# cambyse/po-rrt

Measured on AMD Instinct MI355X. Metric: RRT node-expansions/sec on map_benchmark.pgm, higher is better.
Workload: dtype f64

## Files before the change

### po_rrt_amd/csrc/porrt_device.hpp

```cpp
#pragma once
#include <hip/hip_runtime.h>
#include <stdint.h>
#include <string>
#include <vector>
#include "../../include/porrt_hip.h"

namespace porrt {

template <int NEV>
struct ScopedEvents {
    hipEvent_t e[NEV];
    ScopedEvents() { for (int i = 0; i < NEV; ++i) e[i] = nullptr; }
    hipError_t create() {
        for (int i = 0; i < NEV; ++i) { const hipError_t r = hipEventCreate(&e[i]); if (r != hipSuccess) return r; }
        return hipSuccess;
    }
    ~ScopedEvents() { for (int i = 0; i < NEV; ++i) if (e[i]) (void)hipEventDestroy(e[i]); }
    ScopedEvents(const ScopedEvents &) = delete;
    ScopedEvents &operator=(const ScopedEvents &) = delete;
};

template <class Launch, class GoingOn>
static int sweep_to_fixpoint(hipStream_t stream, uint32_t *flags, size_t rows, int cur, Launch &&launch, GoingOn &&going_on, const char *who,
                             uint64_t &sweeps, std::string &err) {
// ... 66 lines not shown
    uint32_t pend_cnt, pool_n;
    uint32_t n_deferred, pend_lo;
    uint32_t n_losers;
    uint32_t kd_snap;
    uint32_t dbg[4];
    uint32_t clone_n;
    uint32_t clone_k[64];
    uint32_t coop_bar;
    uint32_t coop_filed;
    uint32_t coop_abort;
    uint32_t sched_stop;
    uint32_t sched_iter;
    uint32_t n_lca;
    uint32_t lca_next;
    unsigned long long tim[16];
};

#ifdef PORRT_TIMING
#define PORRT_T0() unsigned long long t__0 = wall_clock64()
#define PORRT_TACC(rc, slot)                                                                          \
    do {                                                                                              \
        const unsigned long long t__1 = wall_clock64();                                               \
        if ((threadIdx.x & 63u) == 0u) { atomicAdd(&(rc).cnt->tim[slot], t__1 - t__0); atomicAdd(&(rc).cnt->tim[(slot) + 8], 1ull); } \
        t__0 = t__1;                                                                                  \
    } while (0)
#else
#define PORRT_T0() do {} while (0)
#define PORRT_TACC(rc, slot) do {} while (0)
#endif
#ifndef PORRT_TIMING_FROM
// ... 757 lines not shown
#else
template <class T> using HitRow = T __attribute__((address_space(1))) *;
template <class T> using LdsPtr = T *;
#endif

__device__ __forceinline__ uint32_t region_of(const RunConst &rc, double x, double y) {
    int cx, cy;
    rep_cell(rc, x, y, kRG, cx, cy);
    return (uint32_t)(cy * kRG + cx);
}

__device__ __forceinline__ double disc_radius(double bound_d2, double qx, double qy) {
    return sqrt(bound_d2) * (1.0 + 1e-9) + 1e-12 * (1.0 + fabs(qx) + fabs(qy));
}

template <bool BUF = false, class Visit>
__device__ __forceinline__ void scan_disc(const RunConst &rc, uint32_t b, double qx, double qy, double rho, uint32_t N, uint32_t lane, Visit visit,
                                          uint32_t skip_region = 0xFFFFFFFFu, uint32_t share = 0u, uint32_t nshare = 1u) {
    int cx0, cy0, cx1, cy1;
    rep_cell(rc, qx - rho, qy - rho, kRG, cx0, cy0);
    rep_cell(rc, qx + rho, qy + rho, kRG, cx1, cy1);
    const uint32_t x0 = uni((uint32_t)cx0), y0 = uni((uint32_t)cy0);
    const uint32_t w = uni((uint32_t)(cx1 - cx0 + 1)), nreg = w * uni((uint32_t)(cy1 - cy0 + 1));
    if (nreg * 16u > N) {
        [[maybe_unused]] auto gx = as_global(rc.nx), gy = as_global(rc.ny);
        for (uint32_t j0 = share * 128u; j0 < N; j0 += nshare * 128u) {
            double x[2], y[2];
#pragma unroll
            for (int u = 0; u < 2; ++u) {
                const uint32_t j = j0 + 64u * u + lane;
                if constexpr (BUF) {
                    x[u] = g_at(rc.nx, (j < N ? j : 0u) * 8u);
                    y[u] = g_at(rc.ny, (j < N ? j : 0u) * 8u);
                } else {
                    x[u] = gx[j < N ? j : 0u];
                    y[u] = gy[j < N ? j : 0u];
                }
            }
#pragma unroll
            for (int u = 0; u < 2; ++u)
                if (j0 + 64u * u < N) visit(x[u], y[u], (int)(j0 + 64u * u + lane), j0 + 64u * u + lane < N);
        }
        return;
    }
    auto gcnt = as_global(rc.rg_cnt) + (b & 1u) * kRegions;
    auto gdir = as_global(rc.rg_dir);
    [[maybe_unused]] auto gxy = as_global(reinterpret_cast<const dbl2 *>(rc.pg_xy));
    [[maybe_unused]] auto gid = as_global(rc.pg_id);
    [[maybe_unused]] PageBuf pb;
    if constexpr (BUF) pb = page_buf(rc);
    for (uint32_t r0 = 0; r0 < nreg; r0 += 64) {
        const uint32_t r = r0 + lane;
        uint32_t reg = 0, cnt = 0;
        if (r < nreg) {
            const uint32_t ry = r / w;
            reg = (y0 + ry) * kRG + x0 + (r - ry * w);
            cnt = reg == skip_region ? 0u : gcnt[reg];
        }
        const uint32_t npg = (uint32_t)__popcll(__ballot(cnt > 0u));
        if (__ballot(cnt >= npg || cnt > kPage) == 0ull && npg > 1u) {
            if (nshare > 1u && r % nshare != share) cnt = 0u;
            uint32_t cmax = cnt;
            for (int off = 32; off > 0; off >>= 1) {
                const uint32_t o = __shfl_xor(cmax, off);
                cmax = o > cmax ? o : cmax;
            }
            cmax = uni(cmax);
            for (uint32_t s0 = 0; s0 < cmax; s0 += 2) {
                dbl2 v[2];
                int id[2];
#pragma unroll
                for (int u = 0; u < 2; ++u) {
                    if constexpr (BUF) {
                        const uint32_t at = s0 + u < cnt ? reg * kPage + s0 + u : kNoSlot;
                        v[u] = page_xy(pb, at);
                        id[u] = page_id(pb, at);
                    } else {
                        const uint32_t sl = s0 + u < cnt ? s0 + u : 0u;
                        v[u] = gxy[(size_t)reg * kPage + sl];
                        id[u] = gid[(size_t)reg * kPage + sl];
                    }
                }
                if constexpr (BUF) __atomic_signal_fence(__ATOMIC_SEQ_CST);
#pragma unroll
                for (int u = 0; u < 2; ++u)
                    if (s0 + u < cmax) visit(v[u].x, v[u].y, id[u], s0 + u < cnt);
            }
            continue;
        }
        uint32_t page = reg;
        for (uint32_t j = 0;; ++j) {
            unsigned long long m = __ballot(cnt > j * kPage);
            if (!m) break;
            if (nshare > 1u) m = __ballot(cnt > j * kPage && (r + j) % nshare == share);
            if (j && cnt > j * kPage) page = gdir[(size_t)reg * rc.rg_maxp + j];
            while (m) {
                uint32_t pg[2], pc[2];
#pragma unroll
                for (int u = 0; u < 2; ++u) {
                    pg[u] = 0; pc[u] = 0;
                    if (m) {
                        const uint32_t l = (uint32_t)__builtin_ctzll(m);
                        m &= m - 1;
                        pg[u] = (uint32_t)__builtin_amdgcn_readlane((int)page, (int)l);
                        const uint32_t c = (uint32_t)__builtin_amdgcn_readlane((int)cnt, (int)l) - j * kPage;
                        pc[u] = c < kPage ? c : kPage;
                    }
                }
                dbl2 v[2];
                int id[2];
#pragma unroll
                for (int u = 0; u < 2; ++u) {
                    const bool ld = lane < pc[u];
                    if constexpr (BUF) {
                        const uint32_t at = ld ? pg[u] * kPage + lane : kNoSlot;
                        v[u] = page_xy(pb, at);
                        id[u] = page_id(pb, at);
                    } else {
                        v[u] = ld ? gxy[(size_t)pg[u] * kPage + lane] : dbl2{0.0, 0.0};
                        id[u] = ld ? gid[(size_t)pg[u] * kPage + lane] : -1;
                    }
                }
                if constexpr (BUF) __atomic_signal_fence(__ATOMIC_SEQ_CST);
#pragma unroll
                for (int u = 0; u < 2; ++u)
                    if (pc[u]) visit(v[u].x, v[u].y, id[u], lane < pc[u]);
            }
        }
    }
}

template <bool PTO>
__device__ __forceinline__ void near_sample(const RunConst &rc, uint32_t b, uint32_t i0, uint32_t vwords, uint32_t k, uint32_t lane) {
    const uint32_t N = uni(as_global(rc.n_at)[b]);
    const double sqx = uni_d(as_global(rc.sx)[i0 + k]), sqy = uni_d(as_global(rc.sy)[i0 + k]);
    uint32_t world = 0;
    if (PTO) world = uni(as_global(rc.sworld)[i0 + k]);
    const double INF = __longlong_as_double(0x7FF0000000000000ll);
    double bestD = INF;
    int best = 0x7FFFFFFF;
    const double T2 = rc.rad_T2[N + (rc.mode == 1 ? 1u : 0u)];
// ... 547 lines not shown
        }
        return v;
    }
};

struct GlobalList {
    static constexpr bool kCompact = false;
    GPTR(const int) cid;
    GPTR(const dbl2) cxy;
    GPTR(double) cval;
    GPTR(const double) gdA;
    __device__ __forceinline__ int id(uint32_t a) const { return cid[a]; }
    __device__ __forceinline__ void xy(uint32_t a, double &x, double &y) const { const dbl2 v = cxy[a]; x = v.x; y = v.y; }
    __device__ __forceinline__ double val(uint32_t a) const { return cval[a]; }
    __device__ __forceinline__ void set_val(uint32_t a, double v) const { cval[a] = v; }
    __device__ __forceinline__ void set_dA(uint32_t, double) const {}
    __device__ __forceinline__ double dA(uint32_t, int j) const { return gdA[j]; }
};
__device__ __forceinline__ GlobalList global_list(const RunConst &rc, uint32_t b, uint32_t k) {
    GlobalList L;
    L.cid = as_global((const int *)rc.cand_id) + cand_off(rc, b, k);
    L.cxy = as_global(reinterpret_cast<const dbl2 *>(rc.cand_xy)) + cand_off(rc, b, k);
    L.cval = as_global(rc.cand_val) + cand_val_off(rc, b, k);
    L.gdA = as_global((const double *)rc.distA);
    return L;
}
#ifndef PORRT_LDS_HITS
#define PORRT_LDS_HITS 80
#endif
constexpr uint32_t kLdsHits = PORRT_LDS_HITS;
// ... 18 lines not shown
    static constexpr bool kCompact = true;
    HitRow<int> sid;
    HitRow<dbl2> sxy;
    HitRow<double> sd;
    HitRow<int> out_id;
    HitRow<double> out_val;
    GPTR(uint32_t) out_cnt;
    uint32_t out_cap;
    __device__ __forceinline__ int id(uint32_t a) const { return sid[a]; }
    __device__ __forceinline__ void xy(uint32_t a, double &x, double &y) const { const dbl2 v = sxy[a]; x = v.x; y = v.y; }
    __device__ __forceinline__ double val(uint32_t a) const { return sxy[a].x; }
    __device__ __forceinline__ void set_val(uint32_t a, double v) const { sxy[a].x = v; }
    __device__ __forceinline__ void set_dA(uint32_t, double) const {}
    __device__ __forceinline__ double dA(uint32_t a, int) const { return sd[a]; }
};

struct NoNearestSearch { __device__ int operator()() const { return 0; } };
template <class TeamT, class ListT, class Grid, class NNF = NoNearestSearch>
__device__ void connect_rrt_sample(const RunConst &rc, const TeamT &tm, const ListT &L, const Grid &grid, uint32_t b, uint32_t k, uint32_t id,
                                   double px, double py, uint32_t cnt, uint32_t &err, const uint32_t *clone_ids = nullptr, uint32_t n_clone = 0,
                                   int clr_known = -1, NNF nearest_search = NNF(), uint32_t swap = 0) {
    const uint32_t tl = tm.tl(), TS = TeamT::kSize;
    const int goal_kind = rc.goal_kind;
    auto gdA = as_global(swap ? rc.distB : rc.distA);
    const double INF = __longlong_as_double(0x7FF0000000000000ll);

    PORRT_T0();
    double bt = INF;
    int bj = 0x7FFFFFFF;
    uint32_t nvalid = 0, leq = 0;
// ... 261 lines not shown
            }
            if (tl == 0) *L.out_cnt = n_out;
        }
        PORRT_TACC_S(rc, 7);
        return;
    } else {
    if (j0 >= 0) {
        double out = -1.0;
        if (nvalid != 0 && cost0 >= 0.0 && j0 != best) {
            const double via = dnew + cost0;
            if (via < dA0) {
                g_atomic_min(gdB + j0, f64_bits(via));
                out = via;
            }
        }
        L.set_val(tl, out);
    }
    for (uint32_t a = tl + TS; a < cnt; a += TS) {
        const double cost = L.val(a);
        const int j = L.id(a);
        double out = -1.0;
        if (nvalid != 0 && cost >= 0.0 && j != best) {
            const double via = dnew + cost;
            if (via < L.dA(a, j)) {
                g_atomic_min(gdB + j, f64_bits(via));
                out = via;
            }
        }
        L.set_val(a, out);
    }
    }
}

constexpr uint32_t kHeavyCand = 256;

template <bool LDSGRID>
__device__ __forceinline__ void connect_block(const RunConst &rc, uint32_t b, uint32_t nb, uint32_t vwords, uint32_t bx, uint8_t *lds_tiles, double *s_d, int *s_i,
                                              uint32_t *s_heavy, uint32_t swap = 0) {
    const uint32_t lane = threadIdx.x & 63u, wv = threadIdx.x >> 6;
    const uint32_t k = uni(bx * kConnectWaves + wv);
    const uint32_t qo = q_off(rc, b);
    const bool active = k < nb && as_global(rc.q_vid)[qo + (k < nb ? k : 0)] >= 0;
    const uint32_t cnt = active ? cand_count(rc, b, k) : 0u;
    const bool heavy = active && cnt > kHeavyCand;
// ... 1549 lines not shown
```

### po_rrt_amd/csrc/porrt_engine.hip

```cpp
#include "../../include/porrt_hip.h"
#include "porrt_host.hpp"
#include "porrt_device.hpp"
#include "porrt_group.hpp"
#include "porrt_belief.hpp"
#include "porrt_dp.hpp"
#include "porrt_prm.hpp"
#include "porrt_edges.hpp"
#include "porrt_refine.hpp"
#include "porrt_refine_batch.hpp"
#include "porrt_reparent.hpp"
#include "porrt_qmdp.hpp"
#include "porrt_policy_graph.hpp"
#include "porrt_join.hpp"
#include "porrt_mm_recipe.hpp"

#include <algorithm>
#include <functional>
#include <chrono>
#include <cmath>
#include <cstdio>
#include <cstring>
#include <string>
#include <system_error>
#include <mutex>
// ... 81 lines not shown
    bool opt_graph = true;
    uint32_t opt_kd_group = 0;
    bool opt_kd_after = false;
    int opt_kd_inline = 0;
    int opt_kd_lazy = 1;
    uint32_t opt_claim_threads = 0;
    int opt_host_ranks = 1;
    int opt_compact = 1;
    uint32_t n_compactions = 0;
    int opt_kd_ride = 0;
    int opt_group_req = -1;
    uint32_t opt_early_wave = 0;
    uint32_t opt_conn_wg_waves = 1;
    bool opt_conn_riders_first = true;
    uint32_t opt_riders_fast = 1;
    uint32_t opt_nn_wg_waves = 4;
    uint32_t opt_commit_flat = 1;
    uint32_t opt_batch_streams = 0;
    int opt_pipeline = 4;
    std::vector<void *> dl_pin;
    std::vector<hipStream_t> dl_streams;
    std::vector<size_t> dl_pin_cap;
    hipStream_t dl_out_stream = nullptr;
    TreeOut *d_tree_out = nullptr;
    size_t d_tree_out_cap = 0;
    uint32_t opt_tree_out_blocks = 4;
    uint32_t opt_fetch_workers = 8;
    bool sub_eager = false;
    int last_launch_mode = 0;
    uint32_t sub_streams_tried = 0;
// ... 555 lines not shown
        return;
    }
    (void)hipEventRecord(ev_steered, stream);
    ev();
    if (GLn) {
        const uint32_t lazy = kd_lazy ? 1u : 0u;
        if (cx.opt_conn_wg_waves == 4u) {
            const uint32_t spb = 256u / GLc;
            const dim3 g2((nb + spb - 1) / spb + 2 + lazy, Q);
            const size_t dyn = conn2_wg4_lds_bytes(GLc);
            with_lanes(GLc, [&](auto gl) { hipLaunchKernelGGL(k_conn2_wg4<decltype(gl)::value>, g2, dim3(256), dyn, stream, rcp, b, nb, vwords, lazy, cx.opt_riders_fast); });
        } else {
            const uint32_t spb = 64u / GLc;
            const dim3 g2((nb + spb - 1) / spb, Q), gr(2 + lazy, Q);
            const size_t dyn = conn2_lds_bytes(GLc);
            if (cx.opt_conn_riders_first) hipLaunchKernelGGL(k_conn2_riders, gr, dim3(256), conn2_riders_lds_bytes(), stream, rcp, b, nb, vwords, lazy, cx.opt_riders_fast);
            with_lanes(GLc, [&](auto gl) { hipLaunchKernelGGL(k_conn2<decltype(gl)::value>, g2, dim3(64), dyn, stream, rcp, b, nb, vwords); });
            if (!cx.opt_conn_riders_first) hipLaunchKernelGGL(k_conn2_riders, gr, dim3(256), conn2_riders_lds_bytes(), stream, rcp, b, nb, vwords, lazy, cx.opt_riders_fast);
        }
    } else if (lds_bytes) hipLaunchKernelGGL(k_connect_rrt<true>, cgrid, cblock, lds_bytes, stream, rcp, b, nb, vwords);
    else hipLaunchKernelGGL(k_connect_rrt<false>, cgrid, cblock, 0, stream, rcp, b, nb, vwords);
    ev();
    commit_pend_b = b; commit_pend_nb = nb;
    kd_last_b = b; kd_last_nb = nb;
    side_active = true;
    if (!cx.opt_kd_after && !kd_lazy && b + 1 - kd_b0 >= kd_group) launch_kd_group();
}

static uint32_t launch_kd_claim(hipStream_t st, const RunConst *rcp, uint32_t Q, uint32_t b0, uint32_t ns, uint32_t K, uint32_t vwords, uint32_t threads) {
    const uint64_t nodes = (uint64_t)ns * K;
    if (Q == 1 && threads == 0) {
        if (nodes <= 2048u) { hipLaunchKernelGGL(k_kd_claim<2048>, dim3(1, 1), dim3(1024), 0, st, rcp, b0, ns, vwords); return kKdfClaimOne2048; }
        hipLaunchKernelGGL(k_kd_claim<kClaimMax>, dim3(1, 1), dim3(1024), 0, st, rcp, b0, ns, vwords);
// ... 4101 lines not shown

int porrt_get_option(const porrt_ctx *c, const char *name, int64_t *value) {
    if (!c || !name || !value) return PORRT_ERR_INVALID;
    if (!strcmp(name, "launch_mode")) *value = c->last_launch_mode;
    else if (!strcmp(name, "pipeline")) *value = c->seq.lag_on ? 4 : (c->seq.pipe_on ? 1 : 0);
    else if (!strcmp(name, "group_lanes")) *value = c->seq.opt_group;
    else if (!strcmp(name, "kd_lazy")) *value = c->seq.kd_lazy ? 1 : 0;
    else if (!strcmp(name, "kd_lca_steps")) *value = (int64_t)c->counters.lca_next;
    else if (!strcmp(name, "compactions")) *value = c->n_compactions;
    else if (!strcmp(name, "kd_built_after")) *value = c->seq.kd_built_after;
    else if (!strcmp(name, "kd_forms_run")) *value = c->seq.kd_forms_run;
    else if (!strcmp(name, "n_heavy")) *value = (int64_t)c->counters.n_heavy;
    else if (!strcmp(name, "conn_wg_waves")) *value = c->opt_conn_wg_waves;
    else if (!strcmp(name, "conn_riders_first")) *value = c->opt_conn_riders_first ? 1 : 0;
    else if (!strcmp(name, "riders_fast")) *value = c->opt_riders_fast;
    else if (!strncmp(name, "tim", 3) && name[3] >= '0' && name[3] <= '9' && atoi(name + 3) < 16) *value = (int64_t)c->counters.tim[atoi(name + 3)];
    else if (!strcmp(name, "nn_wg_waves")) *value = c->opt_nn_wg_waves;
    else if (!strcmp(name, "commit_flat")) *value = c->opt_commit_flat;
    else if (!strcmp(name, "cand_cap")) *value = c->opt_cand_cap;
    else if (!strcmp(name, "edge_per_node")) *value = (int64_t)c->edge_per_node;
    else if (!strcmp(name, "tie_pool_ids")) *value = (int64_t)c->tie_pool_ids;
    else if (!strcmp(name, "tie_pooled_ids")) *value = (int64_t)c->counters.pool_n;
    else if (!strcmp(name, "tie_records")) *value = (int64_t)c->counters.pend_cnt;
    else if (!strcmp(name, "dp_wide_rows")) *value = (int64_t)c->opt_dp_wide_rows;
    else if (!strcmp(name, "dp_levels")) *value = c->dp.valid ? (int64_t)c->dp.levels : 0;
    else if (!strcmp(name, "tamp_streams")) *value = c->opt_tamp_streams;
    else if (!strcmp(name, "tamp_wave")) *value = c->opt_tamp_wave;
    else if (!strcmp(name, "tamp_pool")) *value = c->opt_tamp_pool;
    else if (!strcmp(name, "tamp_search")) *value = c->opt_tamp_search;
    else if (!strcmp(name, "tamp_arena_states")) *value = (int64_t)c->opt_tamp_arena_states;
// ... 41 lines not shown
    }
    else if (!strcmp(name, "batch_streams")) c->opt_batch_streams = (uint32_t)std::max<int64_t>(0, std::min<int64_t>(value, 8));
    else if (!strcmp(name, "kd_after")) c->opt_kd_after = value != 0;
    else if (!strcmp(name, "kd_ride")) c->opt_kd_ride = value != 0;
    else if (!strcmp(name, "kd_lazy")) c->opt_kd_lazy = value == 2 ? 2 : (value != 0);
    else if (!strcmp(name, "kd_claim_threads")) { if (value != 0 && value != 256 && value != 512 && value != 1024) return PORRT_ERR_INVALID; c->opt_claim_threads = (uint32_t)value; }
    else if (!strcmp(name, "kd_inline")) c->opt_kd_inline = value != 0;
    else if (!strcmp(name, "compact_rows")) c->opt_compact = value != 0;
    else if (!strcmp(name, "fetch_workers")) c->opt_fetch_workers = (uint32_t)std::max<int64_t>(1, std::min<int64_t>(value, 32));
    else if (!strcmp(name, "tree_out_blocks")) c->opt_tree_out_blocks = (uint32_t)std::max<int64_t>(1, std::min<int64_t>(value, 1024));
    else if (!strcmp(name, "host_ranks")) { c->opt_host_ranks = value != 0; c->eo.tag = ~0ull; }
    else if (!strcmp(name, "early_wave_steps")) c->opt_early_wave = (uint32_t)std::max<int64_t>(0, std::min<int64_t>(value, 64));
    else if (!strcmp(name, "conn_wg_waves")) { if (value != 1 && value != 4) { c->set_err("conn_wg_waves: 1 or 4"); return PORRT_ERR_INVALID; } c->opt_conn_wg_waves = (uint32_t)value; }
    else if (!strcmp(name, "conn_riders_first")) c->opt_conn_riders_first = value != 0;
    else if (!strcmp(name, "riders_fast")) { if (value != 0 && value != 1) { c->set_err("riders_fast: 0 or 1"); return PORRT_ERR_INVALID; } c->opt_riders_fast = (uint32_t)value; }
    else if (!strcmp(name, "nn_wg_waves")) { if (value != 1 && value != 4) { c->set_err("nn_wg_waves: 1 or 4"); return PORRT_ERR_INVALID; } c->opt_nn_wg_waves = (uint32_t)value; }
    else if (!strcmp(name, "commit_flat")) { if (value != 0 && value != 1) { c->set_err("commit_flat: 0 or 1"); return PORRT_ERR_INVALID; } c->opt_commit_flat = (uint32_t)value; }
    else if (!strcmp(name, "kd_group")) c->opt_kd_group = (uint32_t)std::max<int64_t>(0, std::min<int64_t>(value, 8));
    else if (!strcmp(name, "tamp_streams")) { if (value != 0 && value != 1) { c->set_err("tamp_streams: 0 or 1"); return PORRT_ERR_INVALID; } c->opt_tamp_streams = (int)value; }
    else if (!strcmp(name, "tamp_wave")) { if (value < 1 || value > 65536) { c->set_err("tamp_wave: 1 .. 65536"); return PORRT_ERR_INVALID; } c->opt_tamp_wave = (uint32_t)value; }
    else if (!strcmp(name, "tamp_pool")) { if (value < 1 || value > 4096) { c->set_err("tamp_pool: 1 .. 4096"); return PORRT_ERR_INVALID; } c->opt_tamp_pool = (uint32_t)value; }
    else if (!strcmp(name, "tamp_arena_states")) { if (value < 1024 || value > (1ll << 31)) { c->set_err("tamp_arena_states: 1024 (one row's gather) .. 2^31"); return PORRT_ERR_INVALID; } c->opt_tamp_arena_states = (uint64_t)value; }
    else if (!strcmp(name, "tamp_search")) { if (value < 0 || value > 2) { c->set_err("tamp_search: 0 (BranchAndBound), 1 (AStar), 2 (BranchAndBoundMultipleViewPoints)"); return PORRT_ERR_INVALID; } c->opt_tamp_search = (int)value; }
    else if (!strcmp(name, "prm_rows")) { if (value < 1 || value > 4096) { c->set_err("prm_rows: 1 .. 4096"); return PORRT_ERR_INVALID; } c->opt_prm_rows = (uint32_t)value; }
    else if (!strcmp(name, "prm_xcd_rows")) c->opt_prm_xcd_rows = value != 0;
    else if (!strcmp(name, "policy_max_nodes")) { if (value < 1 || value > (int64_t)kPolMaxNodesLimit) { c->set_err("policy_max_nodes: 1 .. 2^24"); return PORRT_ERR_INVALID; } c->opt_policy_max_nodes = (uint32_t)value; }
    else if (!strcmp(name, "plan_batch_max_belief_nodes")) { if (value < 1 || value > (int64_t)kJoinBeliefNodesLimit) { c->set_err("plan_batch_max_belief_nodes: 1 .. 2^32 - 2"); return PORRT_ERR_INVALID; } c->opt_plan_batch_max_belief_nodes = (uint64_t)value; }
    else if (!strcmp(name, "plan_batch_host_ranks")) c->opt_plan_batch_host_ranks = value != 0;
    else if (!strcmp(name, "mm_plan_batch_max_nodes")) { if (value < 1 || value > (int64_t)kMmBatchNodesLimit) { c->set_err("mm_plan_batch_max_nodes: 1 .. 2^31 - 2"); return PORRT_ERR_INVALID; } c->opt_mm_plan_batch_max_nodes = (uint64_t)value; }
    else if (!strcmp(name, "policy_graph_max_pivots")) { if (value < 0 || value > (int64_t)0x7FFFFFFF) { c->set_err("policy_graph_max_pivots: 0 .. 2^31 - 1"); return PORRT_ERR_INVALID; } c->opt_policy_graph_max_pivots = (uint32_t)value; }
// ... 14 lines not shown
```

### po_rrt_amd/csrc/porrt_group.hpp

```cpp
#pragma once
#include "porrt_device.hpp"
#include "porrt_span.hpp"

namespace porrt {


struct GscanNothingBeside { __device__ __forceinline__ void operator()() const {} };
template <int GL, int R, bool WITHD, class Visit, class Beside = GscanNothingBeside>
__device__ __forceinline__ void gscan_disc(const RunConst &rc, uint32_t b, const GTeam<GL> &tm, double qx, double qy, double rho, uint32_t N, Visit visit,
                                           uint32_t skip_region = 0xFFFFFFFFu, Beside beside = Beside()) {
    const uint32_t gl = tm.gl;
    int cx0, cy0, cx1, cy1;
    rep_cell(rc, qx - rho, qy - rho, kRG, cx0, cy0);
    rep_cell(rc, qx + rho, qy + rho, kRG, cx1, cy1);
    const uint32_t x0 = (uint32_t)cx0, y0 = (uint32_t)cy0;
    const uint32_t w = (uint32_t)(cx1 - cx0 + 1), nreg = w * (uint32_t)(cy1 - cy0 + 1);
    constexpr int U = (int)kPage / GL;
    if (nreg * 16u > N) {
#if !PORRT_PAGE_LOADS
        auto gx = as_global(rc.nx), gy = as_global(rc.ny), gdA = as_global(rc.distA);
#endif
        beside();
        for (uint32_t j0 = 0; j0 < N; j0 += (uint32_t)(U * GL)) {
            double x[U], y[U], d[U];
// ... 628 lines not shown
            const uint32_t slot = atomicAdd(&rc.cnt->clone_n, 1u);
            if (slot < 64u) { rc.cnt->clone_k[slot] = k; qv = 1; }
        }
        as_global(rc.q_vid)[k] = qv;
        as_global(rc.bq_x)[slot] = tx; as_global(rc.bq_y)[slot] = ty; as_global(rc.bq_k)[slot] = qv == 0 ? (uint16_t)k : (uint16_t)0xFFFFu;
        if (valid) atomicOr(&rc.valid_mask[(size_t)b * vwords + (k >> 6)], 1ull << (k & 63u));
        if (err) atomicOr(&rc.cnt->err, err);
    }
}

__host__ __device__ inline size_t conn2_lds_bytes(uint32_t GL) {
    (void)GL;
    return (64u / 16u) * kHitBytes;
}
static_assert(kInsertLds <= kFileLds && kGTrackLds <= kFileLds, "the filing's one-round-trip form is the largest of the riders' scratch areas");
__host__ __device__ inline size_t conn2_riders_lds_bytes() { return kFileLds; }
__host__ __device__ inline size_t conn2_wg4_lds_bytes(uint32_t GL) {
    const size_t a = 4u * conn2_lds_bytes(GL);
    static_assert(kGTrackLds <= 4u * (64u / 16u) * kHitBytes, "g_track_step uses the same bytes");
    static_assert(kFileLds <= 4u * (64u / 16u) * kHitBytes, "file_step_fast uses the same bytes");
    return a > kInsertLds ? a : kInsertLds;
}

__device__ __forceinline__ void rider_file(const RunConst &rc, uint32_t b, uint32_t nb, uint32_t vwords, uint8_t *lds, uint32_t fast) {
    if (fast && nb <= 4u * 256u) file_step_fast<256u, 4u, true>(rc, b, nb, vwords, lds);
    else insert_step_pages<1>(rc, b, nb, vwords, lds);
}
__device__ __forceinline__ void rider_gtrack(const RunConst &rc, uint32_t b, uint32_t nb, uint32_t vwords, uint8_t *lds, uint32_t fast) {
    if (fast) g_track_step<2>(rc, b, nb, vwords, lds);
    else g_track_step<1>(rc, b, nb, vwords, lds);
}
// ... 71 lines not shown
        if (lane == 0) base = atomicAdd(tot, (uint32_t)__popcll(hm));
        const uint32_t pos = uni(base) + (uint32_t)__popcll(hm & ((1ull << lane) - 1ull));
        if (in) {
            if (pos < cap) {
                cid[pos] = jd;
                dbl2 v;
                v.x = x; v.y = y;
                cxy[pos] = v;
            } else {
                over = true;
            }
        }
    }, 0xFFFFFFFFu, wv, kConnectWaves);
    if (over) err |= (uint32_t)ERR_CAND_OVERFLOW;
}

#ifndef PORRT_CLONE_SCAN_WAVES
#define PORRT_CLONE_SCAN_WAVES 4
#endif
__device__ __attribute__((noinline)) void clone_workgroup(const RunConst &rc_arg, uint32_t b, uint32_t vwords, uint32_t N, double T2, uint32_t fast) {
    const RunConst &rc = rc_const(rc_arg);
    __shared__ double s_d[kConnectWaves];
    __shared__ int s_i[kConnectWaves];
    __shared__ uint32_t s_cid[64], s_ck[64];
    __shared__ uint32_t s_tot;
    const uint32_t lane = threadIdx.x & 63u, wv = threadIdx.x >> 6;
    uint32_t err = 0;
    uint32_t n = rc.cnt->clone_n;
    n = n < 64u ? n : 64u;
    if (n == 0) return;
    if (threadIdx.x < n) {
        const uint32_t kc = rc.cnt->clone_k[threadIdx.x];
        s_ck[threadIdx.x] = kc;
        s_cid[threadIdx.x] = N + rank_before(rc, b, vwords, kc);
    }
    __syncthreads();
    if (threadIdx.x == 0) {
        uint32_t lead = 0;
        for (uint32_t t = 1; t < n; ++t) if (s_cid[t] < s_cid[lead]) lead = t;
        const uint32_t ti = s_cid[0], tk = s_ck[0];
        s_cid[0] = s_cid[lead]; s_ck[0] = s_ck[lead]; s_cid[lead] = ti; s_ck[lead] = tk;
        rc.cnt->clone_n = 0;
        s_tot = 0;
    }
    __syncthreads();
    const uint32_t kh = uni(s_ck[0]), idh = uni(s_cid[0]);
    if (threadIdx.x >= 1 && threadIdx.x < n) as_global(rc.cand_cnt)[cand_cnt_at(rc, b, s_ck[threadIdx.x])] = 0u;
    const double pxh = uni_d(as_global(rc.q_x)[kh]), pyh = uni_d(as_global(rc.q_y)[kh]);
    uint32_t hc;
    if (PORRT_CLONE_SCAN_WAVES == 4 && fast) {
        list_scan_waves(rc, b, N, T2, kh, pxh, pyh, lane, wv, &s_tot, err);
        __builtin_amdgcn_fence(__ATOMIC_RELEASE, "workgroup");
        __syncthreads();
        __builtin_amdgcn_fence(__ATOMIC_ACQUIRE, "workgroup");
        const uint32_t tot = s_tot;
        if (threadIdx.x == 0) as_global(rc.cand_cnt)[cand_cnt_at(rc, b, kh)] = tot;
        hc = tot < rc.cand_cap ? tot : rc.cand_cap;
    } else {
        if (wv == 0) {
            list_scan_wave(rc, b, N, T2, kh, pxh, pyh, lane, err);
            __threadfence();
        }
        __syncthreads();
        hc = cand_count(rc, b, kh);
    }
    TableGrid grid;
    grid.p = rc.cls; grid.W = rc.W;
    Team<kConnectWaves> tmh;
    tmh.scr_d = s_d; tmh.scr_i = s_i; tmh.wave = wv; tmh.lane = lane;
    connect_rrt_sample(rc, tmh, global_list(rc, b, kh), grid, b, kh, idh, pxh, pyh, hc, err, s_cid + 1, n - 1u, -1,
                       [&]() { return wave_nn(rc, b, N, pxh, pyh); });
    if (err) atomicOr(&rc.cnt->err, err);
}

__device__ __forceinline__ MemHits mem_hits(const RunConst &rc, uint32_t b, uint32_t k) {
    MemHits M;
#if PORRT_PAGE_LOADS
    M.sid = {rc.cand_id, (uint32_t)cand_off(rc, b, k)};
    M.sxy = {reinterpret_cast<dbl2 *>(rc.cand_xy), (uint32_t)cand_off(rc, b, k)};
    M.sd = {rc.cand_val, (uint32_t)cand_val_off(rc, b, k)};
#else
    M.sid = as_global(rc.cand_id) + cand_off(rc, b, k);
    M.sxy = as_global(reinterpret_cast<dbl2 *>(rc.cand_xy)) + cand_off(rc, b, k);
    M.sd = as_global(rc.cand_val) + cand_val_off(rc, b, k);
#endif
    M.out_id = M.sid;
    M.out_val = M.sd;
// ... 184 lines not shown
    xcd_swizzle(bx, by);
    const RunConst &rc = rc_const(rcp + by);
    CONN2_HOLD(rc, b);
    nb = row_nb(rc, b, nb);
    const uint32_t slot = bx * SPB + threadIdx.x / GL;
    if (bx * SPB >= nb) return;
    const uint32_t N = as_global(rc.n_at)[b];
    const double T2 = as_global(rc.t2_at)[b];
    uint32_t k = 0xFFFFu;
    double px = 0.0, py = 0.0;
    if (slot < nb) { k = as_global(rc.bq_k)[slot]; px = as_global(rc.bq_x)[slot]; py = as_global(rc.bq_y)[slot]; }
    conn2_wave<GL>(rc, b, vwords, N, T2, k, px, py, lds_dyn);
}

__global__ __launch_bounds__(256) __attribute__((amdgpu_waves_per_eu(PORRT_CONN2_WAVES, 8))) void k_conn2_riders(const RunConst *__restrict__ rcp, uint32_t b, uint32_t nb, uint32_t vwords, uint32_t lazy,
                                                                                                                  uint32_t fast) {
    extern __shared__ __attribute__((aligned(16))) uint8_t lds_dyn[];
    const RunConst &rc = rc_const(rcp + blockIdx.y);
    const uint32_t role = blockIdx.x;
    nb = row_nb(rc, b, nb);
    if (nb == 0) return;
    RIDERS_T0();
    if (role == 0) rider_file(rc, b, nb, vwords, lds_dyn, fast);
    else if (lazy && role == 2u) rider_gtrack(rc, b, nb, vwords, lds_dyn, fast);
    else clone_workgroup(rc, b, vwords, as_global(rc.n_at)[b], as_global(rc.t2_at)[b], fast);
    RIDERS_MARK(role);
}

template <int GL>
__global__ __launch_bounds__(256) __attribute__((amdgpu_waves_per_eu(PORRT_CONN2_WAVES, 8))) void k_conn2_wg4(const RunConst *__restrict__ rcp, uint32_t b, uint32_t nb, uint32_t vwords, uint32_t lazy, uint32_t fast) {
    static_assert(GL == 16 || GL == 32 || GL == 64, "group size");
    constexpr uint32_t SPB = 256u / GL;
    extern __shared__ __attribute__((aligned(16))) uint8_t lds_dyn[];
    uint32_t bx = blockIdx.x, by = blockIdx.y;
    const uint32_t ns = lazy ? 3u : 2u;
    const uint32_t role = xcd_swizzle_roles(bx, by, ns);
    const RunConst &rc = rc_const(rcp + by);
    nb = row_nb(rc, b, nb);
    if (nb == 0) return;
    if (role == 0) { rider_file(rc, b, nb, vwords, lds_dyn, fast); return; }
    if (lazy && role == 2u) { rider_gtrack(rc, b, nb, vwords, lds_dyn, fast); return; }
    const uint32_t slot = bx * SPB + threadIdx.x / GL;
    if (role == ns) CONN2_HOLD(rc, b);
    const uint32_t N = as_global(rc.n_at)[b];
    const double T2 = as_global(rc.t2_at)[b];
    uint32_t k = 0xFFFFu;
    double px = 0.0, py = 0.0;
    if (role == ns && slot < nb) { k = as_global(rc.bq_k)[slot]; px = as_global(rc.bq_x)[slot]; py = as_global(rc.bq_y)[slot]; }
    if (role == 1) { clone_workgroup(rc, b, vwords, N, T2, fast); return; }
    conn2_wave<GL>(rc, b, vwords, N, T2, k, px, py, lds_dyn + (threadIdx.x >> 6) * conn2_lds_bytes(GL));
}

template <int GL>
__global__ __launch_bounds__(256) void k_commit2(const RunConst *__restrict__ rcp, uint32_t b, uint32_t nb, uint32_t vwords) {
    const RunConst &rc = rc_const(rcp + blockIdx.y);
    const uint32_t k = (blockIdx.x * 256u + threadIdx.x) / GL;
    if (k < nb && k < row_nb(rc, b, nb)) commit_rrt_sample(rc, b, vwords, k, threadIdx.x % GL, GL);
}
__global__ __launch_bounds__(256) __attribute__((amdgpu_waves_per_eu(8, 8))) void k_commit_flat(const RunConst *__restrict__ rcp, uint32_t b, uint32_t nb, uint32_t vwords) {
    commit_flat_span<256u>(rc_const(rcp + blockIdx.y), b, vwords, nb, blockIdx.x);
}

}
```

Baseline: 358.7 million.

## Keep clone workgroup candidate hit lists in LDS with memory fallback

```diff
diff --git a/po_rrt_amd/csrc/porrt_device.hpp b/po_rrt_amd/csrc/porrt_device.hpp
--- a/po_rrt_amd/csrc/porrt_device.hpp
+++ b/po_rrt_amd/csrc/porrt_device.hpp
@@ -104,6 +104,7 @@
     uint32_t n_lca;
     uint32_t lca_next;
     unsigned long long tim[16];
+    uint32_t clone_lds, clone_mem;
 };
 
 #ifdef PORRT_TIMING
@@ -891,7 +892,7 @@
     return sqrt(bound_d2) * (1.0 + 1e-9) + 1e-12 * (1.0 + fabs(qx) + fabs(qy));
 }
 
-template <bool BUF = false, class Visit>
+template <bool BUF = false, bool WITHD = false, class Visit>
 __device__ __forceinline__ void scan_disc(const RunConst &rc, uint32_t b, double qx, double qy, double rho, uint32_t N, uint32_t lane, Visit visit,
                                           uint32_t skip_region = 0xFFFFFFFFu, uint32_t share = 0u, uint32_t nshare = 1u) {
     int cx0, cy0, cx1, cy1;
@@ -899,24 +900,33 @@
     rep_cell(rc, qx + rho, qy + rho, kRG, cx1, cy1);
     const uint32_t x0 = uni((uint32_t)cx0), y0 = uni((uint32_t)cy0);
     const uint32_t w = uni((uint32_t)(cx1 - cx0 + 1)), nreg = w * uni((uint32_t)(cy1 - cy0 + 1));
+    [[maybe_unused]] auto visit_d = [&](double x, double y, double d, int id, bool ok) {
+        if constexpr (WITHD) visit(x, y, d, id, ok);
+    };
     if (nreg * 16u > N) {
         [[maybe_unused]] auto gx = as_global(rc.nx), gy = as_global(rc.ny);
         for (uint32_t j0 = share * 128u; j0 < N; j0 += nshare * 128u) {
             double x[2], y[2];
+            [[maybe_unused]] double d[2];
 #pragma unroll
             for (int u = 0; u < 2; ++u) {
                 const uint32_t j = j0 + 64u * u + lane;
                 if constexpr (BUF) {
                     x[u] = g_at(rc.nx, (j < N ? j : 0u) * 8u);
                     y[u] = g_at(rc.ny, (j < N ? j : 0u) * 8u);
+                    if constexpr (WITHD) d[u] = g_at(rc.distA, (j < N ? j : 0u) * 8u);
                 } else {
                     x[u] = gx[j < N ? j : 0u];
                     y[u] = gy[j < N ? j : 0u];
+                    if constexpr (WITHD) d[u] = as_global(rc.distA)[j < N ? j : 0u];
                 }
             }
 #pragma unroll
             for (int u = 0; u < 2; ++u)
-                if (j0 + 64u * u < N) visit(x[u], y[u], (int)(j0 + 64u * u + lane), j0 + 64u * u + lane < N);
+                if (j0 + 64u * u < N) {
+                    if constexpr (WITHD) visit_d(x[u], y[u], d[u], (int)(j0 + 64u * u + lane), j0 + 64u * u + lane < N);
+                    else visit(x[u], y[u], (int)(j0 + 64u * u + lane), j0 + 64u * u + lane < N);
+                }
         }
         return;
     }
@@ -946,22 +956,28 @@
             for (uint32_t s0 = 0; s0 < cmax; s0 += 2) {
                 dbl2 v[2];
                 int id[2];
+                [[maybe_unused]] double d[2];
 #pragma unroll
                 for (int u = 0; u < 2; ++u) {
                     if constexpr (BUF) {
                         const uint32_t at = s0 + u < cnt ? reg * kPage + s0 + u : kNoSlot;
                         v[u] = page_xy(pb, at);
                         id[u] = page_id(pb, at);
+                        if constexpr (WITHD) d[u] = page_d(pb, at);
                     } else {
                         const uint32_t sl = s0 + u < cnt ? s0 + u : 0u;
                         v[u] = gxy[(size_t)reg * kPage + sl];
                         id[u] = gid[(size_t)reg * kPage + sl];
+                        if constexpr (WITHD) d[u] = as_global(rc.pg_d)[(size_t)reg * kPage + sl];
                     }
                 }
                 if constexpr (BUF) __atomic_signal_fence(__ATOMIC_SEQ_CST);
 #pragma unroll
                 for (int u = 0; u < 2; ++u)
-                    if (s0 + u < cmax) visit(v[u].x, v[u].y, id[u], s0 + u < cnt);
+                    if (s0 + u < cmax) {
+                        if constexpr (WITHD) visit_d(v[u].x, v[u].y, d[u], id[u], s0 + u < cnt);
+                        else visit(v[u].x, v[u].y, id[u], s0 + u < cnt);
+                    }
             }
             continue;
         }
@@ -986,6 +1002,7 @@
                 }
                 dbl2 v[2];
                 int id[2];
+                [[maybe_unused]] double d[2];
 #pragma unroll
                 for (int u = 0; u < 2; ++u) {
                     const bool ld = lane < pc[u];
@@ -993,15 +1010,20 @@
                         const uint32_t at = ld ? pg[u] * kPage + lane : kNoSlot;
                         v[u] = page_xy(pb, at);
                         id[u] = page_id(pb, at);
+                        if constexpr (WITHD) d[u] = page_d(pb, at);
                     } else {
                         v[u] = ld ? gxy[(size_t)pg[u] * kPage + lane] : dbl2{0.0, 0.0};
                         id[u] = ld ? gid[(size_t)pg[u] * kPage + lane] : -1;
+                        if constexpr (WITHD) d[u] = ld ? as_global(rc.pg_d)[(size_t)pg[u] * kPage + lane] : 0.0;
                     }
                 }
                 if constexpr (BUF) __atomic_signal_fence(__ATOMIC_SEQ_CST);
 #pragma unroll
                 for (int u = 0; u < 2; ++u)
-                    if (pc[u]) visit(v[u].x, v[u].y, id[u], lane < pc[u]);
+                    if (pc[u]) {
+                        if constexpr (WITHD) visit_d(v[u].x, v[u].y, d[u], id[u], lane < pc[u]);
+                        else visit(v[u].x, v[u].y, id[u], lane < pc[u]);
+                    }
             }
         }
     }
@@ -1579,6 +1601,7 @@
     __device__ __forceinline__ void xy(uint32_t a, double &x, double &y) const { const dbl2 v = cxy[a]; x = v.x; y = v.y; }
     __device__ __forceinline__ double val(uint32_t a) const { return cval[a]; }
     __device__ __forceinline__ void set_val(uint32_t a, double v) const { cval[a] = v; }
+    __device__ __forceinline__ void set_out(uint32_t a, double v) const { cval[a] = v; }
     __device__ __forceinline__ void set_dA(uint32_t, double) const {}
     __device__ __forceinline__ double dA(uint32_t, int j) const { return gdA[j]; }
 };
@@ -1627,6 +1650,22 @@
     __device__ __forceinline__ void set_dA(uint32_t, double) const {}
     __device__ __forceinline__ double dA(uint32_t a, int) const { return sd[a]; }
 };
+
+struct TeamLdsHits {
+    static constexpr bool kCompact = false;
+    LdsPtr<int> hid;
+    LdsPtr<double> hx, hy, hd;
+    GPTR(double) cval;
+    __device__ __forceinline__ int id(uint32_t a) const { return hid[a]; }
+    __device__ __forceinline__ void xy(uint32_t a, double &x, double &y) const { x = hx[a]; y = hy[a]; }
+    __device__ __forceinline__ double val(uint32_t a) const { return hx[a]; }
+    __device__ __forceinline__ void set_val(uint32_t a, double v) const { hx[a] = v; }
+    __device__ __forceinline__ void set_out(uint32_t a, double v) const { cval[a] = v; }
+    __device__ __forceinline__ void set_dA(uint32_t, double) const {}
+    __device__ __forceinline__ double dA(uint32_t a, int) const { return hd[a]; }
+};
+constexpr uint32_t kCloneLdsHits = 1216;
+static_assert(kCloneLdsHits % 2u == 0u && kCloneLdsHits * 28u <= 48u * 1024u, "kCloneLdsHits");
 
 struct NoNearestSearch { __device__ int operator()() const { return 0; } };
 template <class TeamT, class ListT, class Grid, class NNF = NoNearestSearch>
@@ -1918,7 +1957,7 @@
                 out = via;
             }
         }
-        L.set_val(tl, out);
+        L.set_out(tl, out);
     }
     for (uint32_t a = tl + TS; a < cnt; a += TS) {
         const double cost = L.val(a);
@@ -1931,7 +1970,7 @@
                 out = via;
             }
         }
-        L.set_val(a, out);
+        L.set_out(a, out);
     }
     }
 }
diff --git a/po_rrt_amd/csrc/porrt_engine.hip b/po_rrt_amd/csrc/porrt_engine.hip
--- a/po_rrt_amd/csrc/porrt_engine.hip
+++ b/po_rrt_amd/csrc/porrt_engine.hip
@@ -119,6 +119,8 @@
     uint32_t opt_conn_wg_waves = 1;
     bool opt_conn_riders_first = true;
     uint32_t opt_riders_fast = 1;
+    int opt_clone_lds_hits = -1;
+    uint32_t clone_cap() const { return opt_clone_lds_hits < 0 ? kCloneLdsHits : (uint32_t)opt_clone_lds_hits; }
     uint32_t opt_nn_wg_waves = 4;
     uint32_t opt_commit_flat = 1;
     uint32_t opt_batch_streams = 0;
@@ -704,9 +706,9 @@
             const uint32_t spb = 64u / GLc;
             const dim3 g2((nb + spb - 1) / spb, Q), gr(2 + lazy, Q);
             const size_t dyn = conn2_lds_bytes(GLc);
-            if (cx.opt_conn_riders_first) hipLaunchKernelGGL(k_conn2_riders, gr, dim3(256), conn2_riders_lds_bytes(), stream, rcp, b, nb, vwords, lazy, cx.opt_riders_fast);
+            if (cx.opt_conn_riders_first) hipLaunchKernelGGL(k_conn2_riders, gr, dim3(256), conn2_riders_lds_bytes(), stream, rcp, b, nb, vwords, lazy, cx.opt_riders_fast, cx.clone_cap());
             with_lanes(GLc, [&](auto gl) { hipLaunchKernelGGL(k_conn2<decltype(gl)::value>, g2, dim3(64), dyn, stream, rcp, b, nb, vwords); });
-            if (!cx.opt_conn_riders_first) hipLaunchKernelGGL(k_conn2_riders, gr, dim3(256), conn2_riders_lds_bytes(), stream, rcp, b, nb, vwords, lazy, cx.opt_riders_fast);
+            if (!cx.opt_conn_riders_first) hipLaunchKernelGGL(k_conn2_riders, gr, dim3(256), conn2_riders_lds_bytes(), stream, rcp, b, nb, vwords, lazy, cx.opt_riders_fast, cx.clone_cap());
         }
     } else if (lds_bytes) hipLaunchKernelGGL(k_connect_rrt<true>, cgrid, cblock, lds_bytes, stream, rcp, b, nb, vwords);
     else hipLaunchKernelGGL(k_connect_rrt<false>, cgrid, cblock, 0, stream, rcp, b, nb, vwords);
@@ -4838,6 +4840,10 @@
     else if (!strcmp(name, "conn_wg_waves")) *value = c->opt_conn_wg_waves;
     else if (!strcmp(name, "conn_riders_first")) *value = c->opt_conn_riders_first ? 1 : 0;
     else if (!strcmp(name, "riders_fast")) *value = c->opt_riders_fast;
+    else if (!strcmp(name, "clone_lds_hits")) *value = c->opt_clone_lds_hits;
+    else if (!strcmp(name, "clone_lds_hits_max")) *value = kCloneLdsHits;
+    else if (!strcmp(name, "clone_lds_steps")) *value = (int64_t)c->counters.clone_lds;
+    else if (!strcmp(name, "clone_mem_steps")) *value = (int64_t)c->counters.clone_mem;
     else if (!strncmp(name, "tim", 3) && name[3] >= '0' && name[3] <= '9' && atoi(name + 3) < 16) *value = (int64_t)c->counters.tim[atoi(name + 3)];
     else if (!strcmp(name, "nn_wg_waves")) *value = c->opt_nn_wg_waves;
     else if (!strcmp(name, "commit_flat")) *value = c->opt_commit_flat;
@@ -4909,6 +4915,10 @@
     else if (!strcmp(name, "conn_wg_waves")) { if (value != 1 && value != 4) { c->set_err("conn_wg_waves: 1 or 4"); return PORRT_ERR_INVALID; } c->opt_conn_wg_waves = (uint32_t)value; }
     else if (!strcmp(name, "conn_riders_first")) c->opt_conn_riders_first = value != 0;
     else if (!strcmp(name, "riders_fast")) { if (value != 0 && value != 1) { c->set_err("riders_fast: 0 or 1"); return PORRT_ERR_INVALID; } c->opt_riders_fast = (uint32_t)value; }
+    else if (!strcmp(name, "clone_lds_hits")) {
+        if (value < -1) { c->set_err("clone_lds_hits: -1 (default), 0 (lists in memory) or a number of entries"); return PORRT_ERR_INVALID; }
+        c->opt_clone_lds_hits = value < 0 ? -1 : (int)std::min<int64_t>(value, (int64_t)kCloneLdsHits);
+    }
     else if (!strcmp(name, "nn_wg_waves")) { if (value != 1 && value != 4) { c->set_err("nn_wg_waves: 1 or 4"); return PORRT_ERR_INVALID; } c->opt_nn_wg_waves = (uint32_t)value; }
     else if (!strcmp(name, "commit_flat")) { if (value != 0 && value != 1) { c->set_err("commit_flat: 0 or 1"); return PORRT_ERR_INVALID; } c->opt_commit_flat = (uint32_t)value; }
     else if (!strcmp(name, "kd_group")) c->opt_kd_group = (uint32_t)std::max<int64_t>(0, std::min<int64_t>(value, 8));
diff --git a/po_rrt_amd/csrc/porrt_group.hpp b/po_rrt_amd/csrc/porrt_group.hpp
--- a/po_rrt_amd/csrc/porrt_group.hpp
+++ b/po_rrt_amd/csrc/porrt_group.hpp
@@ -666,7 +666,9 @@
     return (64u / 16u) * kHitBytes;
 }
 static_assert(kInsertLds <= kFileLds && kGTrackLds <= kFileLds, "the filing's one-round-trip form is the largest of the riders' scratch areas");
-__host__ __device__ inline size_t conn2_riders_lds_bytes() { return kFileLds; }
+constexpr uint32_t kCloneListLds = kCloneLdsHits * (4u + 8u + 8u + 8u);
+static_assert(kCloneListLds <= 48u * 1024u, "the riders' dynamic LDS needs no launch attribute");
+__host__ __device__ inline size_t conn2_riders_lds_bytes() { return kFileLds > kCloneListLds ? kFileLds : kCloneListLds; }
 __host__ __device__ inline size_t conn2_wg4_lds_bytes(uint32_t GL) {
     const size_t a = 4u * conn2_lds_bytes(GL);
     static_assert(kGTrackLds <= 4u * (64u / 16u) * kHitBytes, "g_track_step uses the same bytes");
@@ -768,11 +770,38 @@
     }, 0xFFFFFFFFu, wv, kConnectWaves);
     if (over) err |= (uint32_t)ERR_CAND_OVERFLOW;
 }
+__device__ __forceinline__ TeamLdsHits team_lds_hits(const RunConst &rc, uint32_t b, uint32_t k, uint8_t *lds) {
+    TeamLdsHits H;
+    H.hx = (LdsPtr<double>)lds;
+    H.hy = H.hx + kCloneLdsHits;
+    H.hd = H.hy + kCloneLdsHits;
+    H.hid = (LdsPtr<int>)(H.hd + kCloneLdsHits);
+    H.cval = as_global(rc.cand_val) + cand_val_off(rc, b, k);
+    return H;
+}
+__device__ __forceinline__ void list_scan_waves_lds(const RunConst &rc, uint32_t b, uint32_t N, double T2, uint32_t kh, double pxh, double pyh, uint32_t lane,
+                                                    uint32_t wv, uint32_t *tot, const TeamLdsHits &H, uint32_t cap) {
+    auto cid = as_global(rc.cand_id) + cand_off(rc, b, kh);
+    scan_disc<PORRT_PAGE_LOADS != 0, true>(rc, b, pxh, pyh, disc_radius(T2, pxh, pyh), uni(N), lane, [&](double x, double y, double d, int jd, bool ok) {
+        const bool in = ok && dist2(x, y, pxh, pyh) <= T2;
+        const unsigned long long hm = __ballot(in);
+        if (!hm) return;
+        uint32_t base = 0;
+        if (lane == 0) base = atomicAdd(tot, (uint32_t)__popcll(hm));
+        const uint32_t pos = uni(base) + (uint32_t)__popcll(hm & ((1ull << lane) - 1ull));
+        if (in && pos < cap) {
+            H.hid[pos] = jd; H.hx[pos] = x; H.hy[pos] = y; H.hd[pos] = d;
+            cid[pos] = jd;
+        }
+    }, 0xFFFFFFFFu, wv, kConnectWaves);
+}
 
 #ifndef PORRT_CLONE_SCAN_WAVES
 #define PORRT_CLONE_SCAN_WAVES 4
 #endif
-__device__ __attribute__((noinline)) void clone_workgroup(const RunConst &rc_arg, uint32_t b, uint32_t vwords, uint32_t N, double T2, uint32_t fast) {
+template <bool LDS>
+__device__ __attribute__((noinline)) bool clone_workgroup(const RunConst &rc_arg, uint32_t b, uint32_t vwords, uint32_t N, double T2, uint32_t fast,
+                                                          uint8_t *lds = nullptr, uint32_t lds_cap = 0u) {
     const RunConst &rc = rc_const(rc_arg);
     __shared__ double s_d[kConnectWaves];
     __shared__ int s_i[kConnectWaves];
@@ -782,7 +811,7 @@
     uint32_t err = 0;
     uint32_t n = rc.cnt->clone_n;
     n = n < 64u ? n : 64u;
-    if (n == 0) return;
+    if (n == 0) return true;
     if (threadIdx.x < n) {
         const uint32_t kc = rc.cnt->clone_k[threadIdx.x];
         s_ck[threadIdx.x] = kc;
@@ -794,13 +823,38 @@
         for (uint32_t t = 1; t < n; ++t) if (s_cid[t] < s_cid[lead]) lead = t;
         const uint32_t ti = s_cid[0], tk = s_ck[0];
         s_cid[0] = s_cid[lead]; s_ck[0] = s_ck[lead]; s_cid[lead] = ti; s_ck[lead] = tk;
-        rc.cnt->clone_n = 0;
+        if (!LDS) rc.cnt->clone_n = 0;
         s_tot = 0;
     }
     __syncthreads();
     const uint32_t kh = uni(s_ck[0]), idh = uni(s_cid[0]);
+    const double pxh = uni_d(as_global(rc.q_x)[kh]), pyh = uni_d(as_global(rc.q_y)[kh]);
+    TableGrid grid;
+    grid.p = rc.cls; grid.W = rc.W;
+    Team<kConnectWaves> tmh;
+    tmh.scr_d = s_d; tmh.scr_i = s_i; tmh.wave = wv; tmh.lane = lane;
+    if constexpr (LDS) {
+        lds_cap = lds_cap < rc.cand_cap ? lds_cap : rc.cand_cap;
+        const TeamLdsHits H = team_lds_hits(rc, b, kh, lds);
+        list_scan_waves_lds(rc, b, N, T2, kh, pxh, pyh, lane, wv, &s_tot, H, lds_cap);
+        __syncthreads();
+        const uint32_t tot = s_tot;
+        if (tot > lds_cap) {
+            __builtin_amdgcn_fence(__ATOMIC_RELEASE, "workgroup");
+            __syncthreads();
+            return false;
+        }
+        if (threadIdx.x == 0) {
+            rc.cnt->clone_n = 0;
+            as_global(rc.cand_cnt)[cand_cnt_at(rc, b, kh)] = tot;
+            atomicAdd(&rc.cnt->clone_lds, 1u);
+        }
+        if (threadIdx.x >= 1 && threadIdx.x < n) as_global(rc.cand_cnt)[cand_cnt_at(rc, b, s_ck[threadIdx.x])] = 0u;
+        connect_rrt_sample(rc, tmh, H, grid, b, kh, idh, pxh, pyh, tot, err, s_cid + 1, n - 1u, -1,
+                           [&]() { return wave_nn(rc, b, N, pxh, pyh); });
+    } else {
     if (threadIdx.x >= 1 && threadIdx.x < n) as_global(rc.cand_cnt)[cand_cnt_at(rc, b, s_ck[threadIdx.x])] = 0u;
-    const double pxh = uni_d(as_global(rc.q_x)[kh]), pyh = uni_d(as_global(rc.q_y)[kh]);
+    if (threadIdx.x == 0) atomicAdd(&rc.cnt->clone_mem, 1u);
     uint32_t hc;
     if (PORRT_CLONE_SCAN_WAVES == 4 && fast) {
         list_scan_waves(rc, b, N, T2, kh, pxh, pyh, lane, wv, &s_tot, err);
@@ -818,13 +872,15 @@
         __syncthreads();
         hc = cand_count(rc, b, kh);
     }
-    TableGrid grid;
-    grid.p = rc.cls; grid.W = rc.W;
-    Team<kConnectWaves> tmh;
-    tmh.scr_d = s_d; tmh.scr_i = s_i; tmh.wave = wv; tmh.lane = lane;
     connect_rrt_sample(rc, tmh, global_list(rc, b, kh), grid, b, kh, idh, pxh, pyh, hc, err, s_cid + 1, n - 1u, -1,
                        [&]() { return wave_nn(rc, b, N, pxh, pyh); });
+    }
     if (err) atomicOr(&rc.cnt->err, err);
+    return true;
+}
+__device__ __forceinline__ void rider_clone(const RunConst &rc, uint32_t b, uint32_t vwords, uint32_t N, double T2, uint32_t fast, uint8_t *lds, uint32_t lds_cap) {
+    if (PORRT_CLONE_SCAN_WAVES == 4 && fast && lds_cap && clone_workgroup<true>(rc, b, vwords, N, T2, fast, lds, lds_cap)) return;
+    clone_workgroup<false>(rc, b, vwords, N, T2, fast);
 }
 
 __device__ __forceinline__ MemHits mem_hits(const RunConst &rc, uint32_t b, uint32_t k) {
@@ -1039,7 +1095,7 @@
 }
 
 __global__ __launch_bounds__(256) __attribute__((amdgpu_waves_per_eu(PORRT_CONN2_WAVES, 8))) void k_conn2_riders(const RunConst *__restrict__ rcp, uint32_t b, uint32_t nb, uint32_t vwords, uint32_t lazy,
-                                                                                                                  uint32_t fast) {
+                                                                                                                  uint32_t fast, uint32_t clone_cap) {
     extern __shared__ __attribute__((aligned(16))) uint8_t lds_dyn[];
     const RunConst &rc = rc_const(rcp + blockIdx.y);
     const uint32_t role = blockIdx.x;
@@ -1048,7 +1104,7 @@
     RIDERS_T0();
     if (role == 0) rider_file(rc, b, nb, vwords, lds_dyn, fast);
     else if (lazy && role == 2u) rider_gtrack(rc, b, nb, vwords, lds_dyn, fast);
-    else clone_workgroup(rc, b, vwords, as_global(rc.n_at)[b], as_global(rc.t2_at)[b], fast);
+    else rider_clone(rc, b, vwords, as_global(rc.n_at)[b], as_global(rc.t2_at)[b], fast, lds_dyn, clone_cap);
     RIDERS_MARK(role);
 }
 
@@ -1072,7 +1128,7 @@
     uint32_t k = 0xFFFFu;
     double px = 0.0, py = 0.0;
     if (role == ns && slot < nb) { k = as_global(rc.bq_k)[slot]; px = as_global(rc.bq_x)[slot]; py = as_global(rc.bq_y)[slot]; }
-    if (role == 1) { clone_workgroup(rc, b, vwords, N, T2, fast); return; }
+    if (role == 1) { clone_workgroup<false>(rc, b, vwords, N, T2, fast); return; }
     conn2_wave<GL>(rc, b, vwords, N, T2, k, px, py, lds_dyn + (threadIdx.x >> 6) * conn2_lds_bytes(GL));
 }
 
```

New measurement: 361.7 million, median of 6. Within noise of the previous version (+0.8%).
